# arkCyber/whisper-rust

Hardware: AMD Instinct MI355X
Metric: real-time factor (audio-sec/wall-sec), greedy, 30 s synthetic chunks (higher is better)
Workload: dtype f16 operands / f32 accumulate; 1 GPU; ggml-small-shaped synthetic F16 model, greedy best_of=1 temperature_inc=0, 1 x 30 s 16 kHz f32 chunk per GPU, PCM resident in HBM; flash_attn=False, parallelism=chunk-dp1

## Files before the change

### whisper-rust_amd/csrc/wa_mega.hip

```cpp
#include "wa_device.h"
#include "wa_mega.h"

typedef unsigned long long u64;
#define GAS __attribute__((address_space(1)))
typedef GAS u64 gu64;
typedef GAS unsigned gu32;
typedef const GAS wa_f16 * gch;
typedef const GAS float * gcf;
typedef _Float16 half4v __attribute__((ext_vector_type(4)));
typedef unsigned u32x2 __attribute__((ext_vector_type(2)));
typedef unsigned u32x4 __attribute__((ext_vector_type(4)));

typedef const __attribute__((address_space(4))) wa_mega_args * mg_kargs;
__device__ __forceinline__ mg_kargs mg_uniform(mg_kargs p) {
    const unsigned long long v = (unsigned long long) p;
    const unsigned lo = __builtin_amdgcn_readfirstlane((unsigned) v), hi = __builtin_amdgcn_readfirstlane((unsigned) (v >> 32));
    return (mg_kargs) (((unsigned long long) hi << 32) | lo);
}

#define MG_THREADS 512
#define MG_NW (MG_THREADS / 64)
#define MG_NP3 4
#define MG_SPIN_LIMIT 20000u
#ifndef MG_DEFER
// ... 776 lines not shown
            }
            mg_trace(A, wg == 0 && own && lane == 0, (l * 8 + 1) * 8 + 3, mg_now());
            if (A->dbg && l == MG_WGTRACE_LAYER) mg_trace(A, own && lane == 0, 1024 + wg * 8 + 3, mg_now());
            if (own && !MG_DEFER) t = mg_mk8<Q, NS>(pf, Y.co_w, Y.co_d, Y.co_b, nullptr, d, d, row_d, r_d, 0, lane);
            else if (assisted) t = mg_mk16<Q, 4 * NS>(pf, Y.fc2_w, Y.fc2_d, Y.fc2_b, d, d4, row_d, r_d, 0, lane);
        }
        MG_FRESH();
        if constexpr (CQ) {
            const int qs = mg_slot(wave, MG_EX_X1), sg = mg_seg(d), i0 = qs * sg, i1 = min(d, i0 + sg);
            if (qs >= 0) mg_gather_f32<NP3>(c, mg_edge(A, l, E_X1), i0, i1, lane, xf, 300u + l, A,
                                            wave == 0 ? (wg == 0 ? (l * 8 + 2) * 8 : (A->dbg && l == MG_WGTRACE_LAYER ? 1024 + wg * 8 : -1)) : -1);
            mg_barrier();
            MG_FRESH();
            if (wave == 4) t = mg_mk8<Q, NS>(pf, Y.co_w, Y.co_d, Y.co_b, nullptr, d, d, row_d, r_d, 0, lane);
            else if (wave == 3 || wave >= 6) {
                if (l + 1 >= L) mg_prefetch_logits<NS, Q>(A, pf, have_pf, lane, wave);
                else if (wave == 3) t = mg_mk8<Q, NS>(pf, Ly[l + 1].out_w, Ly[l + 1].out_d, Ly[l + 1].out_b, nullptr, d, d, row_d, r_d, 0, lane);
                else t = mg_mk8<Q, NS>(pf, Ly[l + 1].qkv_w, Ly[l + 1].qkv_d, Ly[l + 1].qkv_b, Ly[l + 1].qkv_s, 3 * d, d, row_qkv, r_qkv, wave - 6, lane);
            }
        } else
        mg_ln3<NP3, Q>(A, c, mg_edge(A, l, E_X1), gw, gb, mg_slot(wave, MG_EX_P4), lane, xf, xinB, lnred, 300u + l,
                       wave == 0 ? (wg == 0 ? (l * 8 + 2) * 8 : (A->dbg && l == MG_WGTRACE_LAYER ? 1024 + wg * 8 : -1)) : -1);
        MG_FRESH();
        if (MG_DEFER && !CQ && wave == 3) t = mg_mk8<Q, NS>(pf, Y.co_w, Y.co_d, Y.co_b, nullptr, d, d, row_d, r_d, 0, lane);
        if (BIGP && wave >= 6 && wave - 2 < g_ff) t = mg_mk8<Q, NS>(pf, Y.fc1_w, Y.fc1_d, Y.fc1_b, nullptr, d4, d, row_ff, r_ff, wave - 2, lane);
        mg_ln_params<NP3>(gw, gb, Y.ln3_w, Y.ln3_b, d, mg_slot(wave, MG_EX_P7), lane);
        if (!CQ && (wave == 4 || (BIG && wave == 3))) {
            const bool own = !BIG || wave == 4;
            bool assisted = false;
            gu64 * eq = mg_edge(A, l, E_QC);
            for (int grp = own ? 0 : 1; grp < g_d8; grp += BIG ? 2 : 1) {
                if (grp >= 1) { t = mg_mk8<Q, NS>(pf, Y.cq_w, Y.cq_d, Y.cq_b, nullptr, d, d, row_d, r_d, grp, lane); assisted = true; }
                MG_CHAOS_AT(3u);
                float v = mg_do8<Q, NS>(pf, t, d >> 5, xinB, lane);
                v = v + t.bias;
                mg_pub_h2(eq, seq, t.valid, t.row, (unsigned) f2h(v), lane);
            }
            mg_trace(A, wg == 0 && own && lane == 0, (l * 8 + 2) * 8 + 3, mg_now());
            if (A->dbg && l == MG_WGTRACE_LAYER) mg_trace(A, own && lane == 0, 1024 + wg * 8 + 6, mg_now());
            if (QB) t = mg_mk8<Q, NS>(pf, Y.fc1_w, Y.fc1_d, Y.fc1_b, nullptr, d4, d, 32 * wg, 32, 3, lane);
            else if (own && !MG_DEFER) {
                if (l + 1 < L) t = mg_mk8<Q, NS>(pf, Ly[l + 1].cq_w, Ly[l + 1].cq_d, Ly[l + 1].cq_b, nullptr, d, d, row_d, r_d, 0, lane);
                else mg_prefetch_logits<NS, Q>(A, pf, have_pf, lane, wave);
            } else if (assisted) t = mg_mk8<Q, NS>(pf, Y.co_w, Y.co_d, Y.co_b, nullptr, d, d, row_d, r_d, 0, lane);
        }
        MG_FRESH();
        {
            const int qs = mg_slot(wave, MG_EX_AO2), sg = mg_seg(Q ? 9 * (d >> 5) : d >> 1), j0 = qs * sg, j1 = min(Q ? 9 * (d >> 5) : d >> 1, j0 + sg);
            if constexpr (Q) { if (qs >= 0) mg_gather_qb<1>(c, mg_edge(A, l, E_AO2), j0, j1, lane, xin, d >> 5, 400u + l, A, wg == 0 && wave == 0 ? (l * 8 + 3) * 8 : -1); }
            else if (qs >= 0) mg_gather_h2<2>(c, mg_edge(A, l, E_AO2), j0, j1, lane, (unsigned *) xin, 400u + l, A, wg == 0 && wave == 0 ? (l * 8 + 3) * 8 : -1);
        }
        mg_barrier();
        MG_FRESH();
        if (MG_DEFER && !QB && !BIGP && !CQ && wave == 4) {
            if (l + 1 < L) t = mg_mk8<Q, NS>(pf, Ly[l + 1].cq_w, Ly[l + 1].cq_d, Ly[l + 1].cq_b, nullptr, d, d, row_d, r_d, 0, lane);
            else mg_prefetch_logits<NS, Q>(A, pf, have_pf, lane, wave);
        }
        if (wave == (CQ ? 4 : 3) || (BIG && wave == 4)) {
            const bool own = !BIG || wave == 3;
            bool assisted = false;
            gu64 * ex = mg_edge(A, l, E_X2);
            for (int grp = own ? 0 : 1; grp < g_d8; grp += BIG ? 2 : 1) {
                if (grp >= 1) { t = mg_mk8<Q, NS>(pf, Y.co_w, Y.co_d, Y.co_b, nullptr, d, d, row_d, r_d, grp, lane); assisted = true; }
                MG_CHAOS_AT(4u);
                float v = mg_do8<Q, NS>(pf, t, d >> 5, xin, lane);
                v = v + t.bias;
                if (t.valid && (lane & 7) == 0) gr_store(ex + t.row, seq, __float_as_uint(v + xf[t.row]));
            }
            mg_trace(A, wg == 0 && own && lane == 0, (l * 8 + 3) * 8 + 3, mg_now());
            if (A->dbg && l == MG_WGTRACE_LAYER) mg_trace(A, own && lane == 0, 4096 + wg * 8 + 3, mg_now());
            if (QB) t = mg_mk8<Q, NS>(pf, Y.fc1_w, Y.fc1_d, Y.fc1_b, nullptr, d4, d, 32 * wg, 32, 2, lane);
            else if (CQ) { if (l + 1 >= L) mg_prefetch_logits<NS, Q>(A, pf, have_pf, lane, wave); }
            else if (BIGP) {
                if (wave - 1 < g_ff) t = mg_mk8<Q, NS>(pf, Y.fc1_w, Y.fc1_d, Y.fc1_b, nullptr, d4, d, row_ff, r_ff, wave - 1, lane);
                else big_next(wave);
            } else if (own && !MG_DEFER) {
                if (l + 1 < L) t = mg_mk8<Q, NS>(pf, Ly[l + 1].out_w, Ly[l + 1].out_d, Ly[l + 1].out_b, nullptr, d, d, row_d, r_d, 0, lane);
                else mg_prefetch_logits<NS, Q>(A, pf, have_pf, lane, wave);
            } else if (assisted) {
                if (l + 1 < L) t = mg_mk8<Q, NS>(pf, Ly[l + 1].cq_w, Ly[l + 1].cq_d, Ly[l + 1].cq_b, nullptr, d, d, row_d, r_d, 0, lane);
                else mg_prefetch_logits<NS, Q>(A, pf, have_pf, lane, wave);
            }
        }
        MG_FRESH();
        if (l == 0 && wave >= 3 && wave <= 5) asm volatile("s_waitcnt vmcnt(0)" ::: "memory");
        mg_ln3<NP3, Q>(A, c, mg_edge(A, l, E_X2), gw, gb, mg_slot(wave, MG_EX_P7), lane, xf, xinB, lnred, 500u + l,
                       wave == 0 ? (wg == 0 ? (l * 8 + 4) * 8 : (A->dbg && l == MG_WGTRACE_LAYER ? 4096 + wg * 8 : -1)) : -1);
        MG_FRESH();
        if (MG_DEFER && !QB && !BIGP && !CQ && wave == 3) {
            if (l + 1 < L) t = mg_mk8<Q, NS>(pf, Ly[l + 1].out_w, Ly[l + 1].out_d, Ly[l + 1].out_b, nullptr, d, d, row_d, r_d, 0, lane);
            else mg_prefetch_logits<NS, Q>(A, pf, have_pf, lane, wave);
        }
        if (l + 1 < L) mg_ln_params<NP3>(gw, gb, Ly[l + 1].ln1_w, Ly[l + 1].ln1_b, d, mg_slot(wave, MG_EX_P1), lane);
        else           mg_ln_params<NP3>(gw, gb, A->lnf_w, A->lnf_b, d, mg_slot(wave, MG_EX_FINAL), lane);
        if (QB) {
            if (wave >= 1 && wave <= 4) {
                MG_CHAOS_AT(5u);
                float v = mg_do8<Q, NS>(pf, t, d >> 5, xinB, lane);
                v = v + t.bias;
                float gl = v;
                if (v <= -10.0f) gl = 0.0f; else if (v < 10.0f) gl = h2f(gelu_l[t.valid ? f2h(v) : 0]);
                if ((lane & 7) == 0) fc1x[8 * (wave - 1) + (lane >> 3)] = gl;
                MG_CHAOS_AT(51u);
                unsigned arrived = 0;
                asm volatile("s_waitcnt lgkmcnt(0)" ::: "memory");
                if (lane == 0) arrived = __hip_atomic_fetch_add(fc1cnt, 1u, __ATOMIC_RELAXED, __HIP_MEMORY_SCOPE_WORKGROUP);
                arrived = (unsigned) __builtin_amdgcn_readfirstlane((int) arrived);
                asm volatile("" ::: "memory");
                if ((arrived & 3u) == 3u && 32 * wg < d4) {
                    MG_CHAOS_AT(52u);
                    const float y = fc1x[lane & 31];
                    float a = fabsf(y);
                    a = fmaxf(a, dpp_f32<0x128>(a)); a = fmaxf(a, dpp_f32<0x124>(a)); a = fmaxf(a, dpp_f32<0x122>(a)); a = fmaxf(a, dpp_f32<0x121>(a));
                    a = fmaxf(a, __shfl_xor(a, 16, 32));
                    const float dq = a / 127.f, id = a != 0.0f ? 127.f / a : 0.0f;
                    const unsigned q = (unsigned) (int) rintf(y * id) & 0xffu;
                    const unsigned w = q | (dpp_u32<0x101>(q) << 8) | (dpp_u32<0x102>(q) << 16) | (dpp_u32<0x103>(q) << 24);
                    gu64 * eb = mg_edge(A, l, E_HF) + (size_t) wg * 9;
                    if (lane < 32 && (lane & 3) == 0) gr_store(eb + (lane >> 2), seq, w);
                    if (lane == 0) gr_store(eb + 8, seq, __float_as_uint(h2f(f2h(dq))));
                    mg_trace(A, wg == 0 && lane == 0, (l * 8 + 4) * 8 + 3, mg_now());
                }
                if (wave == 3) {
                    if (l + 1 < L) t = mg_mk8<Q, NS>(pf, Ly[l + 1].out_w, Ly[l + 1].out_d, Ly[l + 1].out_b, nullptr, d, d, row_d, r_d, 0, lane);
                    else mg_prefetch_logits<NS, Q>(A, pf, have_pf, lane, wave);
                } else if (wave == 4) {
                    if (l + 1 < L) t = mg_mk8<Q, NS>(pf, Ly[l + 1].cq_w, Ly[l + 1].cq_d, Ly[l + 1].cq_b, nullptr, d, d, row_d, r_d, 0, lane);
                    else mg_prefetch_logits<NS, Q>(A, pf, have_pf, lane, wave);
                }
            }
        } else if (BIGP) {
            if ((wave >= 1 && wave <= 4) || wave >= 6) {
                gu64 * eh = mg_edge(A, l, E_HF);
                for (int grp = wave <= 4 ? wave - 1 : wave - 2; grp < g_ff; grp += 6) {
                    if (grp >= 6) t = mg_mk8<Q, NS>(pf, Y.fc1_w, Y.fc1_d, Y.fc1_b, nullptr, d4, d, row_ff, r_ff, grp, lane);
                    MG_CHAOS_AT(6u);
                    float v = mg_do8<Q, NS>(pf, t, d >> 5, xinB, lane);
                    v = v + t.bias;
                    float gl = v;
                    if (v <= -10.0f) gl = 0.0f; else if (v < 10.0f) gl = h2f(gelu_l[t.valid ? f2h(v) : 0]);
                    if constexpr (Q) { if (t.valid && (lane & 7) == 0) gr_store(eh + t.row, seq, __float_as_uint(gl)); }
                    else mg_pub_h2(eh, seq, t.valid, t.row, (unsigned) f2h(gl), lane);
                }
                mg_trace(A, wg == 0 && wave == 1 && lane == 0, (l * 8 + 4) * 8 + 3, mg_now());
                if ((wave == 3 || wave == 4) && wave - 1 < g_ff) big_next(wave);
                else if (wave >= 6 && l + 1 >= L) mg_prefetch_logits<NS, Q>(A, pf, have_pf, lane, wave);
            }
        } else
        if (wave == 1 || wave == 2 || (BIG && (wave == 3 || wave == 4))) {
            const bool own = !BIG || wave <= 2;
            bool assisted = false;
            gu64 * eh = mg_edge(A, l, E_HF);
            for (int grp = wave - 1; grp < g_ff; grp += BIG ? 4 : 2) {
                if (grp >= 2) { t = mg_mk8<Q, NS>(pf, Y.fc1_w, Y.fc1_d, Y.fc1_b, nullptr, d4, d, row_ff, r_ff, grp, lane); assisted = true; }
                MG_CHAOS_AT(7u);
                float v = mg_do8<Q, NS>(pf, t, d >> 5, xinB, lane);
                v = v + t.bias;
                float gl = v;
                if (v <= -10.0f) gl = 0.0f; else if (v < 10.0f) gl = h2f(gelu_l[t.valid ? f2h(v) : 0]);
                if constexpr (Q) { if (t.valid && (lane & 7) == 0) gr_store(eh + t.row, seq, __float_as_uint(gl)); }
                else mg_pub_h2(eh, seq, t.valid, t.row, (unsigned) f2h(gl), lane);
            }
            mg_trace(A, wg == 0 && wave == 1 && lane == 0, (l * 8 + 4) * 8 + 3, mg_now());
            if (A->dbg && l == MG_WGTRACE_LAYER) mg_trace(A, wave == 1 && lane == 0, 4096 + wg * 8 + 6, mg_now());
            if (own && !MG_DEFER) {
                if (l + 1 < L) t = mg_mk8<Q, NS>(pf, Ly[l + 1].qkv_w, Ly[l + 1].qkv_d, Ly[l + 1].qkv_b, Ly[l + 1].qkv_s, 3 * d, d, row_qkv, r_qkv, wave - 1, lane);
                else mg_prefetch_logits<NS, Q>(A, pf, have_pf, lane, wave);
            } else if (CQ) {
                if (l + 1 >= L) mg_prefetch_logits<NS, Q>(A, pf, have_pf, lane, wave);
            } else if (assisted) {
                if (l + 1 >= L) mg_prefetch_logits<NS, Q>(A, pf, have_pf, lane, wave);
                else t = wave == 3 ? mg_mk8<Q, NS>(pf, Ly[l + 1].out_w, Ly[l + 1].out_d, Ly[l + 1].out_b, nullptr, d, d, row_d, r_d, 0, lane)
                                   : mg_mk8<Q, NS>(pf, Ly[l + 1].cq_w, Ly[l + 1].cq_d, Ly[l + 1].cq_b, nullptr, d, d, row_d, r_d, 0, lane);
            }
        }
        MG_FRESH();
        {
            const int ng = QB ? 9 * (d4 >> 5) : Q ? d4 : 2 * d;
            const int qs = mg_slot(wave, QB || BIGP ? MG_EX_HFQ : MG_EX_HF), sg = mg_seg(ng), i0 = qs * sg, i1 = min(ng, i0 + sg);
            if constexpr (QB) { if (qs >= 0) mg_gather_qb<3>(c, mg_edge(A, l, E_HF), i0, i1, lane, xin, d4 >> 5, 600u + l, A, wg == 0 && wave == 0 ? (l * 8 + 5) * 8 : -1); }
            else if constexpr (Q) { if (qs >= 0) mg_gather_q8<(NP3 == MG_NP3 ? 14 : 8)>(c, mg_edge(A, l, E_HF), i0, i1, lane, xin, d4 >> 5, 600u + l, A, wg == 0 && wave == 0 ? (l * 8 + 5) * 8 : -1); }
            else if (qs >= 0) mg_gather_h2<7>(c, mg_edge(A, l, E_HF), i0, i1, lane, (unsigned *) xin, 600u + l, A, wg == 0 && wave == 0 ? (l * 8 + 5) * 8 : -1);
        }
        mg_barrier();
        MG_FRESH();
        mg_trace(A, wg == 0 && wave == 5 && lane == 0, (l * 8 + 5) * 8 + 4, mg_now());
        if (MG_DEFER && !CQ && (wave == 1 || wave == 2)) {
            if (l + 1 < L) t = mg_mk8<Q, NS>(pf, Ly[l + 1].qkv_w, Ly[l + 1].qkv_d, Ly[l + 1].qkv_b, Ly[l + 1].qkv_s, 3 * d, d, row_qkv, r_qkv, wave - 1, lane);
            else mg_prefetch_logits<NS, Q>(A, pf, have_pf, lane, wave);
        }
        if (wave == 5 || (BIG && (wave == 3 || wave == 4))) {
            const bool own = !BIG || wave == 5;
            bool assisted = false;
            gu64 * ex = mg_edge(A, l, E_X3);
            for (int grp = own ? 0 : wave - 2; grp < g_d16; grp += BIG ? 3 : 1) {
                if (grp >= (BIGP ? 3 : 1)) t = mg_mk16<Q, 4 * NS>(pf, Y.fc2_w, Y.fc2_d, Y.fc2_b, d, d4, row_d, r_d, grp, lane);
                if (grp >= 1) assisted = true;
                MG_CHAOS_AT(8u);
                float v = mg_do16<Q, 4 * NS>(pf, t, d4 >> 5, xin, lane);
                v = v + t.bias;
                if (t.valid && (lane & 15) == MG_RES16(Q)) gr_store(ex + t.row, seq, __float_as_uint(v + xf[t.row]));
            }
            mg_trace(A, wg == 0 && own && lane == 0, (l * 8 + 5) * 8 + 3, mg_now());
            if (own && (!MG_DEFER || l + 1 >= L)) {
                if (l + 1 < L) t = mg_mk16<Q, 4 * NS>(pf, Ly[l + 1].fc2_w, Ly[l + 1].fc2_d, Ly[l + 1].fc2_b, d, d4, row_d, r_d, 0, lane);
                else mg_prefetch_logits<NS, Q>(A, pf, have_pf, lane, wave);
            } else if (assisted) {
                if (l + 1 >= L) mg_prefetch_logits<NS, Q>(A, pf, have_pf, lane, wave);
                else t = wave == 3 ? mg_mk8<Q, NS>(pf, Ly[l + 1].out_w, Ly[l + 1].out_d, Ly[l + 1].out_b, nullptr, d, d, row_d, r_d, 0, lane)
                                   : mg_mk8<Q, NS>(pf, Ly[l + 1].cq_w, Ly[l + 1].cq_d, Ly[l + 1].cq_b, nullptr, d, d, row_d, r_d, 0, lane);
            }
        }
    }
    if (L == 0 && wave >= 1 && wave <= 5) mg_prefetch_logits<NS, Q>(A, pf, have_pf, lane, wave);
    MG_FRESH();
    mg_final<NP3, NS, Q>(A, c, smem, pf, have_pf, gw, gb, lane, wave);
#undef MG_FRESH
}

struct mg_att_smem { float * sc; wa_f16 * p16; float * gs; float * red; double * redd; float * s_inv; wa_f16 * qs; float * part; };
__device__ __forceinline__ mg_att_smem mg_att_carve(unsigned char * base, int maxkv) {
    mg_att_smem m;
    m.redd = (double *) base;                       base += 8 * sizeof(double);
    m.sc   = (float *) base;                        base += (size_t) maxkv * 4;
    m.gs   = (float *) base;                        base += (size_t) (maxkv / 8) * 4;
    m.part = (float *) base;                        base += 32 * 64 * 4;
    m.red  = (float *) base;                        base += 8 * 4;
    m.s_inv = (float *) base;                       base += 4 * 4;
    m.p16  = (wa_f16 *) base;                       base += (size_t) maxkv * 2;
    m.qs   = (wa_f16 *) base;
    return m;
}


__device__ __forceinline__ float mg_score(const u32x4 & ka, const u32x4 & kb, const float (&qa)[8], const float (&qb)[8], float scale) {
    const wa_f16 * k8a = (const wa_f16 *) &ka, * k8b = (const wa_f16 *) &kb;
    float v[8];
#pragma unroll
    for (int l = 0; l < 8; ++l) {
        float t = fmaf(h2f(k8a[l]), qa[l], 0.0f);
        t = fmaf(h2f(k8b[l]), qb[l], t);
        t = t + dpp_f32<0x4e>(t);
        v[l] = t + dpp_f32<0xb1>(t);
    }
    const float t0 = v[0] + v[4], t1 = v[1] + v[5], t2 = v[2] + v[6], t3 = v[3] + v[7];
    return ((t0 + t1) + (t2 + t3)) * scale;
}

template <bool Q = false>
__device__ __forceinline__ void mg_attn_finish(const float * part, const wa_f16 * vleft , const wa_f16 * p16, int np, int nl,
                                               gu64 * edge, int h, unsigned seq, int tid, double * dbl0, double * dbl1 ,
                                               mg_kargs A = nullptr, int tslot = -1) {
    asm volatile("" : "+s"(nl));
    if (tid >= 64) {
        const int wv = tid >> 6, o = tid & 63;
        float nzero = -0.0f;
        asm volatile("" : "+v"(nzero));
#pragma unroll
        for (int i = 0; i < 5; ++i) {
            const int cc = 5 * (wv - 1) + i;
            if (cc < 32) {
                const float pr = fmaf(h2f(vleft[cc * 64 + o]), h2f((p16 + np)[cc]), nzero);
                (cc < 16 ? dbl0 : dbl1)[(cc & 15) * 64 + o] = (double) (cc < nl ? pr : -0.0f);
            }
        }
    }
    double sumf = 0.0;
    if (tid < 64) {
        if (tslot >= 0) mg_trace(A, tid == 0, tslot, mg_now());
        float s32[32];
#pragma unroll
        for (int r = 0; r < 32; ++r) s32[r] = part[r * 64 + tid];
        sumf = (double) wa_tree32(s32);
        if (tslot >= 0) mg_trace(A, tid == 0, tslot + 1, mg_now() + (sumf == 1e300 ? 1u : 0u));
    }
    mg_barrier();
    if (tid < 64) {
        double dv[32];
#pragma unroll
        for (int cc = 0; cc < 32; ++cc) dv[cc] = (cc < 16 ? dbl0 : dbl1)[(cc & 15) * 64 + tid];
        __builtin_amdgcn_sched_barrier(0);
#pragma unroll
        for (int cc = 0; cc < 32; ++cc) sumf += dv[cc];
        if (tslot >= 0) mg_trace(A, tid == 0, tslot + 2, mg_now() + (sumf == 1e300 ? 1u : 0u));
        if constexpr (Q) {
            const float y = (float) sumf;
            float a = fabsf(y);
            a = fmaxf(a, dpp_f32<0x128>(a)); a = fmaxf(a, dpp_f32<0x124>(a)); a = fmaxf(a, dpp_f32<0x122>(a)); a = fmaxf(a, dpp_f32<0x121>(a));
            a = fmaxf(a, __shfl_xor(a, 16, 32));
            const float dsc = a / 127.f, id = a != 0.0f ? 127.f / a : 0.0f;
            const unsigned q = (unsigned) (int) rintf(y * id) & 0xffu;
            const unsigned w = q | (dpp_u32<0x101>(q) << 8) | (dpp_u32<0x102>(q) << 16) | (dpp_u32<0x103>(q) << 24);
            gu64 * eb = edge + (size_t) (2 * h + (tid >> 5)) * 9;
            if ((tid & 3) == 0) gr_store(eb + ((tid & 31) >> 2), seq, w);
            if ((tid & 31) == 0) gr_store(eb + 8, seq, __float_as_uint(h2f(f2h(dsc))));
        } else {
        const unsigned hv = (unsigned) f2h((float) sumf);
        const unsigned hi = dpp_u32<0x101>(hv);
        if ((tid & 1) == 0) gr_store(edge + ((h * 64 + tid) >> 1), seq, (hv & 0xffffu) | (hi << 16));
        }
    }
}

template <bool Q = false>
__device__ __forceinline__ void mg_role_self(mg_kargs A_, int idx_) {
    extern __shared__ __attribute__((aligned(16))) unsigned char smem[];
    const mg_kargs A = mg_uniform(A_);
    const int tid = threadIdx.x, lane = tid & 63;
    const int wave = __builtin_amdgcn_readfirstlane(tid >> 6);
    const int h = __builtin_amdgcn_readfirstlane(idx_);
    mg_ctl c; c.status = (gu32 *) A->status; c.seq = A->seq; c.dead = false;
    mg_chaos_start(c.seq);

    wa_f16 * Ks = (wa_f16 *) smem;
    wa_f16 * Vs = Ks + WA_MEGA_MAX_KV * 64;
    const mg_att_smem M = mg_att_carve(smem + (size_t) WA_MEGA_MAX_KV * 64 * 2 * 2, WA_MEGA_MAX_KV);
    const int d = A->d, n_kv = A->n_kv, kv_head = A->kv_head, L = A->n_layer;
    const int a = tid & 3, kslot = tid >> 2;
    if (wave == 0) mg_pick(A, lane, (int *) (smem + MG_PICK_OFF));
    for (int l = 0; l < L; ++l) {
        {
            const gch kc = (gch) A->kv_k + (size_t) l * A->kv_layer_stride + h * 64;
            const gch vc = (gch) A->kv_v + (size_t) l * A->kv_layer_stride + h * 64;
            const int n16 = n_kv * 8;
            u32x4 tk[8], tv[8];
#pragma unroll
            for (int j = 0; j < 8; ++j) {
                const int idx = tid + MG_THREADS * j;
                if (idx < n16) {
                    tk[j] = *(const GAS u32x4 *) (kc + (size_t) (idx >> 3) * d + (idx & 7) * 8);
                    tv[j] = *(const GAS u32x4 *) (vc + (size_t) (idx >> 3) * d + (idx & 7) * 8);
                }
            }
#pragma unroll
            for (int j = 0; j < 8; ++j) {
                const int idx = tid + MG_THREADS * j;
                if (idx < n16) { *(u32x4 *) (Ks + (size_t) idx * 8) = tk[j]; *(u32x4 *) (Vs + (size_t) idx * 8) = tv[j]; }
            }
        }
        mg_barrier();
        if (wave == 0) {
            unsigned v[2];
            const unsigned sp = mg_sweep<2>(mg_edge(A, l, E_QKV), [&](int k) {
                if (k == 0) return (lane < 32 ? 0 : (d >> 1)) + h * 32 + (lane & 31);
                return lane < 32 ? d + h * 32 + lane : -1; }, c, lane, v, 1000u + l);
            mg_trace(A, h == 0 && lane == 0, (l * 8 + 6) * 8 + 0, mg_now()); mg_trace(A, h == 0 && lane == 0, (l * 8 + 6) * 8 + 1, sp);
            if (lane < 32) { ((unsigned *) M.qs)[lane] = v[0]; ((unsigned *) (Vs + (size_t) kv_head * 64))[lane] = v[1]; }
            else ((unsigned *) (Ks + (size_t) kv_head * 64))[lane - 32] = v[0];
        }
        mg_barrier();
        float lmax = -INFINITY;
        {
            float qa[8], qb[8];
#pragma unroll
            for (int i = 0; i < 8; ++i) { qa[i] = h2f(M.qs[8 * a + i]); qb[i] = h2f(M.qs[32 + 8 * a + i]); }
            for (int c0 = 0; c0 < n_kv; c0 += MG_THREADS / 4) {
                const int cc = c0 + kslot, cl = cc < n_kv ? cc : n_kv - 1;
                const u32x4 ka = *(const u32x4 *) (Ks + (size_t) cl * 64 + 8 * a), kb = *(const u32x4 *) (Ks + (size_t) cl * 64 + 32 + 8 * a);
                const float r = mg_score(ka, kb, qa, qb, 1.0f);
                if (cc < n_kv) { if (a == 0) M.sc[cc] = r; lmax = fmaxf(lmax, r); }
            }
        }
        mg_trace(A, h == 0 && tid == 0, (l * 8 + 6) * 8 + 4, mg_now());
        {
            lmax = wave_max(lmax);
            if (lane == 0) M.red[wave] = lmax;
            mg_barrier();
            float mx = M.red[0];
#pragma unroll
            for (int k = 1; k < MG_NW; ++k) mx = fmaxf(mx, M.red[k]);
            const int n8 = n_kv & ~7, ng = n8 >> 3;
            float e = 0.0f;
            double ps = 0.0;
            if (tid < n_kv) e = tid < n8 ? wa_expf(M.sc[tid] - mx) : wa_expf_libm(M.sc[tid] - mx);
            {
                float t = e + dpp_f32<0x104>(e);
                t = t + dpp_f32<0x102>(t);
                t = t + dpp_f32<0x101>(t);
                if (tid < n8) ps = (tid & 7) == 0 ? (double) t : 0.0;
                else if (tid < n_kv) ps = (double) e;
            }
            ps = wave_sum_d(ps);
            if (lane == 0) M.redd[wave] = ps;
            mg_barrier();
            const double tot = ((M.redd[0] + M.redd[1]) + (M.redd[2] + M.redd[3])) + ((M.redd[4] + M.redd[5]) + (M.redd[6] + M.redd[7]));
            const double delta = (double) (ng + 8 + 16) * 0x1p-53 * tot * 1.000001;
            const float ilo = (float) (1.0 / (tot + delta)), ihi = (float) (1.0 / (tot - delta));
            if (ilo != ihi && tid == 0 && !c.dead) __hip_atomic_store(c.status, (unsigned) WA_MEGA_REDO, __ATOMIC_RELAXED, __HIP_MEMORY_SCOPE_AGENT);
            if (tid < n_kv) M.p16[tid] = f2h(e * ilo);
            mg_barrier();
        }
        mg_trace(A, h == 0 && tid == 0, (l * 8 + 6) * 8 + 5, mg_now());
        MG_CHAOS_ID(1000 + h, 21u, c.seq);
        const int np = n_kv & ~31, nsteps = np >> 5;
        {
            float acc[4] = { 0.0f, 0.0f, 0.0f, 0.0f };
            const int r0 = wave * 4;
            for (int s = 0; s < nsteps; ++s) {
#pragma unroll
                for (int i = 0; i < 4; ++i)
                    acc[i] = fmaf(h2f(Vs[(size_t) (s * 32 + r0 + i) * 64 + lane]), h2f(M.p16[s * 32 + r0 + i]), acc[i]);
            }
#pragma unroll
            for (int i = 0; i < 4; ++i) M.part[(r0 + i) * 64 + lane] = acc[i];
        }
        mg_barrier();
        mg_attn_finish<Q>(M.part, Vs + (size_t) np * 64, M.p16, np, n_kv - np, mg_edge(A, l, E_AO), h, c.seq, tid, (double *) (Ks + WA_MEGA_KV_ROOM * 64),
                          (double *) (Vs + WA_MEGA_KV_ROOM * 64), A, A->dbg && h == 0 && l == MG_WGTRACE_LAYER ? 3004 : -1);
        mg_trace(A, h == 0 && tid == 0, (l * 8 + 6) * 8 + 3, mg_now());
        mg_barrier();
    }
    unsigned pf[96];
    bool have_pf = false;
    float gw[MG_NP3], gb[MG_NP3];
    if (wave >= 1) mg_prefetch_logits<0, Q>(A, pf, have_pf, lane, wave);
    mg_ln_params<MG_NP3>(gw, gb, A->lnf_w, A->lnf_b, A->d, mg_slot(wave, MG_EX_FINAL), lane);
    mg_final<MG_NP3, 0, Q>(A, c, smem, pf, have_pf, gw, gb, lane, wave);
}

#define MG_CSTEPS 48
#define MG_CGR 2048
#define MG_CGR_MAX 0
#define MG_CGR_SUM 8
#define MG_CGR_XCC 16
#define MG_CGR_PART 64
#define MG_CX_XF 32768
#define MG_CX_XIN (MG_CX_XF + WA_MEGA_MAX_D * 4)
#define MG_CX_LNRED (MG_CX_XIN + WA_MEGA_MAX_D * 2)
#define MG_CX_END (MG_CX_LNRED + 256)
#define MG_CX_TRACE 6144

template <bool Q = false, int CQ = -1>
__device__ __forceinline__ void mg_role_cross(mg_kargs A_, int idx_) {
    extern __shared__ __attribute__((aligned(16))) unsigned char smem[];
    const mg_kargs A = mg_uniform(A_);
    int tid = threadIdx.x, lane = tid & 63;
    const int wave = __builtin_amdgcn_readfirstlane(tid >> 6);
    const int H = A->n_head;
    const int ci = __builtin_amdgcn_readfirstlane(idx_);
    const int h = ci >> 2, w = ci & 3;
    mg_ctl c; c.status = (gu32 *) A->status; c.seq = A->seq; c.dead = false;
    mg_chaos_start(c.seq);
    const unsigned seq = c.seq;

    float  * part  = (float *) smem;
    wa_f16 * vleft = (wa_f16 *) (smem + 8192);
    float  * sc    = (float *) (smem + 8192 + 4096);
    wa_f16 * p16   = (wa_f16 *) (smem + 8192 + 4096 + 1536);
    wa_f16 * pleft = (wa_f16 *) (smem + 8192 + 4096 + 1536 + 768);
    wa_f16 * qs    = (wa_f16 *) (smem + 8192 + 4096 + 1536 + 768 + 64);
    double * redd  = (double *) (smem + 8192 + 4096 + 1536 + 768 + 64 + 128);
    float  * red   = (float *) (smem + 8192 + 4096 + 1536 + 768 + 64 + 128 + 64);
    float  * bc    = red + 8;

    const int T = A->T, tpad = A->cross_tpad, L = A->n_layer;
    const float kq_scale = A->kq_scale;
    int a = tid & 3, ks = tid >> 2;
    const int np = T & ~31, nsteps = np >> 5, nl = T - np, n8 = T & ~7, ng = n8 >> 3;
    if (wave == 0) mg_pick(A, lane, (int *) (smem + MG_PICK_OFF));
    if (wave == 0) {
        const unsigned xcc = (unsigned) __builtin_amdgcn_s_getreg(20 | (3 << 11)) & 0xfu;
        gu64 * X0 = (gu64 *) A->cross_gr + (size_t) h * MG_CGR + MG_CGR_XCC;
        if (lane == 0) gr_store(X0 + w, seq, xcc);
        unsigned v[1];
        mg_sweep<1>(X0, [&](int) { return lane < 4 ? lane : -1; }, c, lane, v, 2900u);
        const bool same = lane >= 4 || v[0] == xcc;
        if (lane == 0) bc[2] = __builtin_amdgcn_ballot_w64(same) == ~0ull && !c.dead ? 1.0f : 0.0f;
    }
    mg_barrier();
    const bool local = bc[2] != 0.0f;
    const __attribute__((address_space(4))) wa_mega_layer * Ly = (const __attribute__((address_space(4))) wa_mega_layer *) A->layers;
    float  * xf    = (float *) (smem + MG_CX_XF);
    wa_f16 * xin   = (wa_f16 *) (smem + MG_CX_XIN);
    double * lnred = (double *) (smem + MG_CX_LNRED);
    const int d = A->d;
    for (int l = 0; l < L; ++l) {
        if constexpr (CQ >= 0) {
            unsigned z = threadIdx.x; asm volatile("" : "+v"(z));
            tid = (int) z; lane = tid & 63; a = tid & 3; ks = tid >> 2;
        }
        gu64 * X = (gu64 *) A->cross_gr + ((size_t) l * H + h) * MG_CGR;
        const gch kp = (gch) A->cross_k + (size_t) l * A->cross_layer_stride + (size_t) h * tpad * 64;
        const gch vp = (gch) A->cross_v + (size_t) l * A->cross_layer_stride + (size_t) h * tpad * 64;
        u32x4 ka[3], kb[3];
        unsigned short vv[MG_CSTEPS];
#pragma unroll
        for (int p = 0; p < 3; ++p) {
            const int o = p * 128 + ks, cc = 32 * (o >> 3) + 8 * w + (o & 7);
            if (cc < T) { ka[p] = *(const GAS u32x4 *) (kp + (size_t) cc * 64 + 8 * a); kb[p] = *(const GAS u32x4 *) (kp + (size_t) cc * 64 + 32 + 8 * a); }
        }
#pragma unroll
        for (int s = 0; s < MG_CSTEPS; ++s) if (s < nsteps) vv[s] = *(const GAS unsigned short *) (vp + (size_t) (32 * s + 8 * w + wave) * 64 + lane);
        if (w == 0 && tid < 256) {
            const int row = tid >> 3;
            if (row < nl) *(u32x4 *) (vleft + (size_t) tid * 8) = *(const GAS u32x4 *) (vp + (size_t) (np + row) * 64 + (tid & 7) * 8);
        }
        if constexpr (CQ >= 0) {
            unsigned pf[96];
            float gw[2], gb[2];
            const int row = 64 * h + 8 * wave + (lane >> 3);
            const gch wrow = (gch) Ly[l].cq_w + (size_t) row * d + 4 * (lane & 7);
            mg_pf8<CQ>(pf, wrow, true, d >> 5, 0);
            const float bias = ((gcf) Ly[l].cq_b)[row];
            mg_ln_params<2>(gw, gb, Ly[l].ln2_w, Ly[l].ln2_b, d, mg_slot(wave, 0u), lane);
            mg_trace(A, ci == 0 && lane == 0 && wave == 0, (l * 8 + 7) * 8 + 2, mg_now());
            mg_ln3<2>(A, c, mg_edge(A, l, E_X1), gw, gb, mg_slot(wave, 0u), lane, xf, xin, lnred, 2000u + l,
                      ci == 0 && wave == 0 ? MG_CX_TRACE + l * 8 : -1);
            MG_CHAOS_ID(2000 + ci, 30u, seq);
            float v = mg_dot8<CQ>(pf, wrow, true, d >> 5, xin, lane & 7, true);
            v = v + bias;
            const unsigned hq = (unsigned) f2h(v);
            if ((lane & 7) == 0) qs[8 * wave + (lane >> 3)] = (wa_f16) hq;
            if (A->dbg && w == 0) mg_pub_h2(mg_edge(A, l, E_QC), seq, true, row, hq, lane);
            mg_trace(A, ci == 0 && lane == 0 && wave == 0, (l * 8 + 7) * 8 + 0, mg_now());
            if (A->dbg && l == MG_WGTRACE_LAYER && w == 0) mg_trace(A, tid == 0, 3200 + h, mg_now());
        } else if (wave == 0) {
            unsigned v[1];
            mg_trace(A, ci == 0 && lane == 0, (l * 8 + 7) * 8 + 2, mg_now());
            const unsigned sp = mg_sweep<1>(mg_edge(A, l, E_QC), [&](int) { return lane < 32 ? h * 32 + lane : -1; }, c, lane, v, 2000u + l);
            mg_trace(A, ci == 0 && lane == 0, (l * 8 + 7) * 8 + 0, mg_now()); mg_trace(A, ci == 0 && lane == 0, (l * 8 + 7) * 8 + 1, sp);
            if (A->dbg && l == MG_WGTRACE_LAYER && w == 0) mg_trace(A, lane == 0, 3200 + h, mg_now());
            if (lane < 32) ((unsigned *) qs)[lane] = v[0];
        }
        mg_barrier();
#define MG_CX(k) do { if (A->dbg && l == MG_WGTRACE_LAYER) mg_trace(A, ci == 0 && tid == 0, 3010 + (k), mg_now()); } while (0)
        MG_CX(0);
        MG_CHAOS_ID(2000 + ci, 31u, seq);
        float lmax = -INFINITY;
        {
            float qa[8], qb[8];
#pragma unroll
            for (int i = 0; i < 8; ++i) { qa[i] = h2f(qs[8 * a + i]); qb[i] = h2f(qs[32 + 8 * a + i]); }
#pragma unroll
            for (int p = 0; p < 3; ++p) {
                const int o = p * 128 + ks, cc = 32 * (o >> 3) + 8 * w + (o & 7);
                const float r = mg_score(ka[p], kb[p], qa, qb, kq_scale);
                if (cc < T) { if (a == 0) sc[o] = r; lmax = fmaxf(lmax, r); }
            }
        }
        lmax = wave_max(lmax);
        if (lane == 0) red[wave] = lmax;
        MG_CX(1);
        mg_barrier();
        MG_CX(2);
        if (wave == 0) {
            float m = red[0];
#pragma unroll
            for (int k = 1; k < MG_NW; ++k) m = fmaxf(m, red[k]);
            if (lane == 0) gr_store_l(X + MG_CGR_MAX + w, seq, __float_as_uint(m), local);
            unsigned v[1];
            mg_sweep<1>(X + MG_CGR_MAX, [&](int) { return lane < 4 ? lane : -1; }, c, lane, v, 2100u + l);
            float g = lane < 4 ? __uint_as_float(v[0]) : -INFINITY;
            g = fmaxf(g, dpp_f32<0x4e>(g)); g = fmaxf(g, dpp_f32<0xb1>(g));
            if (lane == 0) bc[0] = g;
            MG_CX(3);
        }
        mg_barrier();
        mg_trace(A, ci == 0 && tid == 0, (l * 8 + 7) * 8 + 4, mg_now());
        const float mx = bc[0];
        {
            double ps = 0.0;
            if (tid < 8 * MG_CSTEPS) {
                const int g = 4 * (tid >> 3) + w, cc = 8 * g + (tid & 7);
                const float e = cc < n8 ? wa_expf(sc[tid] - mx) : (cc < T ? wa_expf_libm(sc[tid] - mx) : 0.0f);
                sc[tid] = e;
                float t = e + dpp_f32<0x104>(e);
                t = t + dpp_f32<0x102>(t);
                t = t + dpp_f32<0x101>(t);
                if (g < ng) ps = (tid & 7) == 0 ? (double) t : 0.0;
                else ps = (double) e;
            }
            ps = wave_sum_d(ps);
            if (lane == 0) redd[wave] = ps;
        }
        MG_CX(4);
        mg_barrier();
        if (wave == 0) {
            const double ps = ((redd[0] + redd[1]) + (redd[2] + redd[3])) + ((redd[4] + redd[5]) + (redd[6] + redd[7]));
            const u64 pb = (u64) __double_as_longlong(ps);
            if (lane == 0) { gr_store_l(X + MG_CGR_SUM + 2 * w, seq, (unsigned) pb, local); gr_store_l(X + MG_CGR_SUM + 2 * w + 1, seq, (unsigned) (pb >> 32), local); }
            unsigned v[1];
            mg_sweep<1>(X + MG_CGR_SUM, [&](int) { return lane < 8 ? lane : -1; }, c, lane, v, 2200u + l);
            double tot = 0.0;
#pragma unroll
            for (int k = 0; k < 4; ++k) {
                const unsigned lo = __builtin_amdgcn_readlane(v[0], 2 * k), hi = __builtin_amdgcn_readlane(v[0], 2 * k + 1);
                tot += __longlong_as_double((long long) (((u64) hi << 32) | lo));
            }
            const double delta = (double) (ng + 8 + 16) * 0x1p-53 * tot * 1.000001;
            const float ilo = (float) (1.0 / (tot + delta)), ihi = (float) (1.0 / (tot - delta));
            if (ilo != ihi && lane == 0 && !c.dead) __hip_atomic_store(c.status, (unsigned) WA_MEGA_REDO, __ATOMIC_RELAXED, __HIP_MEMORY_SCOPE_AGENT);
            if (lane == 0) bc[1] = ilo;
            MG_CX(5);
        }
        mg_barrier();
        mg_trace(A, ci == 0 && tid == 0, (l * 8 + 7) * 8 + 5, mg_now());
        const float inv = bc[1];
        if (tid < 8 * MG_CSTEPS) {
            const int cc = 32 * (tid >> 3) + 8 * w + (tid & 7);
            if (cc < T) {
                const wa_f16 ph = f2h(sc[tid] * inv);
                p16[(tid & 7) * MG_CSTEPS + (tid >> 3)] = ph;
                if (cc >= np) { if (w == 0) pleft[cc - np] = ph; else gr_store_l(X + MG_CGR_PART + (w - 1) * 576 + 512 + (tid & 7), seq, (unsigned) ph, local); }
            }
        }
        mg_barrier();
        MG_CX(6);
        MG_CHAOS_ID(2000 + ci, 32u, seq);
        {
            float acc = 0.0f;
            half8 pw[MG_CSTEPS / 8];
#pragma unroll
            for (int k = 0; k < MG_CSTEPS / 8; ++k) pw[k] = *(const half8 *) (p16 + wave * MG_CSTEPS + 8 * k);
#pragma unroll
            for (int s = 0; s < MG_CSTEPS; ++s) if (s < nsteps) acc = fmaf(h2f(vv[s]), (float) pw[s >> 3][s & 7], acc);
            if (w == 0) part[wave * 64 + lane] = acc;
            else gr_store_l(X + MG_CGR_PART + (w - 1) * 576 + wave * 64 + lane, seq, __float_as_uint(acc), local);
        }
        mg_trace(A, ci == 0 && tid == 0, (l * 8 + 7) * 8 + 6, mg_now());
        if (w == 0) {
            if (wave >= 1 && wave <= 6) {
                const int ww = (wave - 1) >> 1, half = (wave - 1) & 1;
                gu64 * src = X + MG_CGR_PART + ww * 576;
                unsigned v[5];
                mg_sweep<5>(src, [&](int k) { return k < 4 ? half * 256 + 64 * k + lane : (half == 0 && lane < 8 && 8 * (ww + 1) + lane < nl ? 512 + lane : -1); }, c, lane, v, 2300u + l);
#pragma unroll
                for (int k = 0; k < 4; ++k) part[(8 * (ww + 1) + 4 * half + k) * 64 + lane] = __uint_as_float(v[k]);
                if (half == 0 && lane < 8) { const int cc = 8 * (ww + 1) + lane; if (cc < nl) pleft[cc] = (wa_f16) v[4]; }
            }
            mg_barrier();
            mg_trace(A, ci == 0 && tid == 0, (l * 8 + 7) * 8 + 7, mg_now());
            mg_attn_finish<Q>(part, vleft, pleft - np, np, nl, mg_edge(A, l, E_AO2), h, seq, tid, (double *) (smem + 16384), (double *) (smem + 24576), A,
                              A->dbg && ci == 0 && l == MG_WGTRACE_LAYER ? 3000 : -1);
            mg_trace(A, ci == 0 && tid == 0, (l * 8 + 7) * 8 + 3, mg_now());
            if (A->dbg && l == MG_WGTRACE_LAYER) mg_trace(A, tid == 0, 3100 + h, mg_now());
        }
        mg_barrier();
    }
    unsigned pf[96];
    bool have_pf = false;
    float gw[MG_NP3], gb[MG_NP3];
    if (wave >= 1) mg_prefetch_logits<0, Q>(A, pf, have_pf, lane, wave);
    mg_ln_params<MG_NP3>(gw, gb, A->lnf_w, A->lnf_b, A->d, mg_slot(wave, MG_EX_FINAL), lane);
    mg_final<MG_NP3, 0, Q>(A, c, smem, pf, have_pf, gw, gb, lane, wave);
}

#ifndef MG_CQ_TU
__global__ __launch_bounds__(MG_THREADS) void k_decode_mega(const wa_mega_args A) {
    int role, idx;
    mg_role_of((int) gridDim.x, A.n_head, (int) blockIdx.x, role, idx);
    const mg_kargs Ap = (mg_kargs) __builtin_amdgcn_kernarg_segment_ptr();
    if (role == 0) {
        if (A.d == 768) mg_role_gemv<2, 24>(Ap, idx); else if (A.d < 768) mg_role_gemv<2, 0>(Ap, idx);
        else mg_role_gemv<MG_NP3, 0>(Ap, idx);
    }
    else if (role == 1) mg_role_self(Ap, idx);
    else                mg_role_cross(Ap, idx);
}


__global__ __launch_bounds__(MG_THREADS) void k_decode_mega_q(const wa_mega_args A) {
    int role, idx;
    mg_role_of((int) gridDim.x, A.n_head, (int) blockIdx.x, role, idx);
    const mg_kargs Ap = (mg_kargs) __builtin_amdgcn_kernarg_segment_ptr();
    if (role == 0) {
        if (A.d == 768) mg_role_gemv<2, 24, true>(Ap, idx); else if (A.d < 768) mg_role_gemv<2, 0, true>(Ap, idx);
        else if (A.d == 1280) mg_role_gemv<MG_NP3, 40, true>(Ap, idx); else mg_role_gemv<MG_NP3, 0, true>(Ap, idx);
    }
    else if (role == 1) mg_role_self<true>(Ap, idx);
    else                mg_role_cross<true>(Ap, idx);
}

size_t wa_mega_lds_bytes() {
    const size_t s_self  = (size_t) WA_MEGA_MAX_KV * 64 * 2 * 2 + MG_ATT_SMEM(WA_MEGA_MAX_KV);
    const size_t s_cross = MG_CX_END;
    const size_t s_gemv  = MG_PICK_OFF;
    size_t m = s_self > s_cross ? s_self : s_cross;
    m = m > s_gemv ? m : s_gemv;
    if (m > MG_PICK_OFF || (MG_PICK_OFF & 255) != 0) abort();
    return MG_PICK_OFF + MG_PICK_BYTES;
}

bool wa_launch_decode_mega(hipStream_t s, const wa_mega_args & a, int n_wg) {
    static bool attr_set[64] = {};
    const size_t lds = wa_mega_lds_bytes();
    int dev = 0;
    (void) hipGetDevice(&dev);
    if (!attr_set[dev & 63]) {
        if (hipFuncSetAttribute((const void *) k_decode_mega, hipFuncAttributeMaxDynamicSharedMemorySize, (int) lds) != hipSuccess ||
            hipFuncSetAttribute((const void *) k_decode_mega_q, hipFuncAttributeMaxDynamicSharedMemorySize, (int) lds) != hipSuccess) return false;
        attr_set[dev & 63] = true;
    }
    if (MG_DEFER && !a.quant && a.d == 768) return wa_launch_decode_mega_cq(s, a, n_wg, lds);
    if (a.quant) hipLaunchKernelGGL(k_decode_mega_q, dim3(n_wg), dim3(MG_THREADS), lds, s, a);
    else         hipLaunchKernelGGL(k_decode_mega, dim3(n_wg), dim3(MG_THREADS), lds, s, a);
    return hipGetLastError() == hipSuccess;
}
#else
__global__ __launch_bounds__(MG_THREADS) void k_decode_mega_cq(const wa_mega_args A) {
    int role, idx;
    mg_role_of((int) gridDim.x, A.n_head, (int) blockIdx.x, role, idx);
    const mg_kargs Ap = (mg_kargs) __builtin_amdgcn_kernarg_segment_ptr();
    if (role == 0)      mg_role_gemv<2, 24, false, true>(Ap, idx);
    else if (role == 1) mg_role_self(Ap, idx);
    else                mg_role_cross<false, 24>(Ap, idx);
}

bool wa_launch_decode_mega_cq(hipStream_t s, const wa_mega_args & a, int n_wg, size_t lds) {
    static bool attr_set[64] = {};
    int dev = 0;
    (void) hipGetDevice(&dev);
    if (!attr_set[dev & 63]) {
        if (hipFuncSetAttribute((const void *) k_decode_mega_cq, hipFuncAttributeMaxDynamicSharedMemorySize, (int) lds) != hipSuccess) return false;
        attr_set[dev & 63] = true;
    }
    hipLaunchKernelGGL(k_decode_mega_cq, dim3(n_wg), dim3(MG_THREADS), lds, s, a);
    return hipGetLastError() == hipSuccess;
}
#endif
```

Baseline: 350.5 x real-time.

## Split cross-attention V columns across the four workgroups to need one exchange

```diff
diff --git a/whisper-rust_amd/csrc/wa_mega.hip b/whisper-rust_amd/csrc/wa_mega.hip
--- a/whisper-rust_amd/csrc/wa_mega.hip
+++ b/whisper-rust_amd/csrc/wa_mega.hip
@@ -1102,6 +1102,28 @@
     }
 }
 
+__device__ __forceinline__ void mg_attn_finish16(const float * part, const double * dbl, gu64 * edge, int o0, unsigned seq, int tid,
+                                                 mg_kargs A = nullptr, int tslot = -1) {
+    if (tid < 16) {
+        if (tslot >= 0) mg_trace(A, tid == 0, tslot, mg_now());
+        float s32[32];
+        double dv[32];
+#pragma unroll
+        for (int r = 0; r < 32; ++r) s32[r] = part[r * 16 + tid];
+#pragma unroll
+        for (int cc = 0; cc < 32; ++cc) dv[cc] = dbl[cc * 16 + tid];
+        __builtin_amdgcn_sched_barrier(0);
+        double sumf = (double) wa_tree32(s32);
+        if (tslot >= 0) mg_trace(A, tid == 0, tslot + 1, mg_now() + (sumf == 1e300 ? 1u : 0u));
+#pragma unroll
+        for (int cc = 0; cc < 32; ++cc) sumf += dv[cc];
+        if (tslot >= 0) mg_trace(A, tid == 0, tslot + 2, mg_now() + (sumf == 1e300 ? 1u : 0u));
+        const unsigned hv = (unsigned) f2h((float) sumf);
+        const unsigned hi = dpp_u32<0x101>(hv);
+        if ((tid & 1) == 0) gr_store(edge + ((o0 + tid) >> 1), seq, (hv & 0xffffu) | (hi << 16));
+    }
+}
+
 template <bool Q = false>
 __device__ __forceinline__ void mg_role_self(mg_kargs A_, int idx_) {
     extern __shared__ __attribute__((aligned(16))) unsigned char smem[];
@@ -1224,14 +1246,17 @@
 #define MG_CGR_SUM 8
 #define MG_CGR_XCC 16
 #define MG_CGR_PART 64
+#define MG_CGR_XCC1 WA_MEGA_MAX_T
+#define MG_CP_LD 56
 #define MG_CX_XF 32768
 #define MG_CX_XIN (MG_CX_XF + WA_MEGA_MAX_D * 4)
 #define MG_CX_LNRED (MG_CX_XIN + WA_MEGA_MAX_D * 2)
 #define MG_CX_END (MG_CX_LNRED + 256)
 #define MG_CX_TRACE 6144
 
-template <bool Q = false, int CQ = -1>
+template <bool Q = false, int CQ = -1, bool X1 = false>
 __device__ __forceinline__ void mg_role_cross(mg_kargs A_, int idx_) {
+    static_assert(!X1 || (CQ >= 0 && !Q), "the one-exchange form is the F16 d = 768 kernel's");
     extern __shared__ __attribute__((aligned(16))) unsigned char smem[];
     const mg_kargs A = mg_uniform(A_);
     int tid = threadIdx.x, lane = tid & 63;
@@ -1252,6 +1277,23 @@
     double * redd  = (double *) (smem + 8192 + 4096 + 1536 + 768 + 64 + 128);
     float  * red   = (float *) (smem + 8192 + 4096 + 1536 + 768 + 64 + 128 + 64);
     float  * bc    = red + 8;
+    double * dbl   = nullptr;
+    if constexpr (X1) {
+        constexpr int o_sc = 0, o_p16 = o_sc + WA_MEGA_MAX_T * 4, o_part = o_p16 + 32 * MG_CP_LD * 2, o_dbl = o_part + 32 * 16 * 4, o_vleft = o_dbl + 32 * 16 * 8,
+                      o_pleft = o_vleft + 32 * 16 * 2, o_qs = o_pleft + 32 * 2, o_redd = o_qs + 64 * 2, o_red = o_redd + 8 * 8, o_bc = o_red + 8 * 4, o_end = o_bc + 4 * 4;
+        static_assert(o_end <= MG_CX_XF && o_p16 % 16 == 0 && o_dbl % 8 == 0 && o_vleft % 16 == 0 && o_redd % 8 == 0 && MG_CP_LD % 8 == 0 && MG_CP_LD >= MG_CSTEPS,
+                      "LDS of the one-exchange form: below the role's LayerNorm area, 16-byte rows where 16 bytes are read");
+        sc    = (float *) (smem + o_sc);
+        p16   = (wa_f16 *) (smem + o_p16);
+        part  = (float *) (smem + o_part);
+        dbl   = (double *) (smem + o_dbl);
+        vleft = (wa_f16 *) (smem + o_vleft);
+        pleft = (wa_f16 *) (smem + o_pleft);
+        qs    = (wa_f16 *) (smem + o_qs);
+        redd  = (double *) (smem + o_redd);
+        red   = (float *) (smem + o_red);
+        bc    = (float *) (smem + o_bc);
+    }
 
     const int T = A->T, tpad = A->cross_tpad, L = A->n_layer;
     const float kq_scale = A->kq_scale;
@@ -1260,7 +1302,7 @@
     if (wave == 0) mg_pick(A, lane, (int *) (smem + MG_PICK_OFF));
     if (wave == 0) {
         const unsigned xcc = (unsigned) __builtin_amdgcn_s_getreg(20 | (3 << 11)) & 0xfu;
-        gu64 * X0 = (gu64 *) A->cross_gr + (size_t) h * MG_CGR + MG_CGR_XCC;
+        gu64 * X0 = (gu64 *) A->cross_gr + (size_t) h * MG_CGR + (X1 ? MG_CGR_XCC1 : MG_CGR_XCC);
         if (lane == 0) gr_store(X0 + w, seq, xcc);
         unsigned v[1];
         mg_sweep<1>(X0, [&](int) { return lane < 4 ? lane : -1; }, c, lane, v, 2900u);
@@ -1289,11 +1331,20 @@
             const int o = p * 128 + ks, cc = 32 * (o >> 3) + 8 * w + (o & 7);
             if (cc < T) { ka[p] = *(const GAS u32x4 *) (kp + (size_t) cc * 64 + 8 * a); kb[p] = *(const GAS u32x4 *) (kp + (size_t) cc * 64 + 32 + 8 * a); }
         }
+        if constexpr (X1) {
+#pragma unroll
+            for (int s = 0; s < MG_CSTEPS; ++s) if (s < nsteps) vv[s] = *(const GAS unsigned short *) (vp + (size_t) (32 * s + (tid >> 4)) * 64 + 16 * w + (tid & 15));
+            if (wave == 0) {
+                const int row = tid >> 1;
+                if (row < nl) *(u32x4 *) (vleft + (size_t) tid * 8) = *(const GAS u32x4 *) (vp + (size_t) (np + row) * 64 + 16 * w + (tid & 1) * 8);
+            }
+        } else {
 #pragma unroll
         for (int s = 0; s < MG_CSTEPS; ++s) if (s < nsteps) vv[s] = *(const GAS unsigned short *) (vp + (size_t) (32 * s + 8 * w + wave) * 64 + lane);
         if (w == 0 && tid < 256) {
             const int row = tid >> 3;
             if (row < nl) *(u32x4 *) (vleft + (size_t) tid * 8) = *(const GAS u32x4 *) (vp + (size_t) (np + row) * 64 + (tid & 7) * 8);
+        }
         }
         if constexpr (CQ >= 0) {
             unsigned pf[96];
@@ -1324,6 +1375,107 @@
         }
         mg_barrier();
 #define MG_CX(k) do { if (A->dbg && l == MG_WGTRACE_LAYER) mg_trace(A, ci == 0 && tid == 0, 3010 + (k), mg_now()); } while (0)
+        if constexpr (X1) {
+        MG_CX(0);
+        MG_CHAOS_ID(2000 + ci, 31u, seq);
+        float lmax = -INFINITY;
+        {
+            float qa[8], qb[8];
+#pragma unroll
+            for (int i = 0; i < 8; ++i) { qa[i] = h2f(qs[8 * a + i]); qb[i] = h2f(qs[32 + 8 * a + i]); }
+#pragma unroll
+            for (int p = 0; p < 3; ++p) {
+                const int o = p * 128 + ks, cc = 32 * (o >> 3) + 8 * w + (o & 7);
+                const float r = mg_score(ka[p], kb[p], qa, qb, kq_scale);
+                if (cc < T) {
+                    if (a == 0) { gr_store_l(X + cc, seq, __float_as_uint(r), local); sc[cc] = r; }
+                    lmax = fmaxf(lmax, r);
+                }
+            }
+        }
+        MG_CX(1);
+        MG_CHAOS_ID(2000 + ci, 33u, seq);
+        {
+            unsigned v[3];
+            const auto other = [&](int k) { const int cg = tid + 512 * k; return cg < T && ((cg >> 3) & 3) != w ? cg : -1; };
+            mg_sweep<3>(X, other, c, lane, v, 2400u + l);
+#pragma unroll
+            for (int k = 0; k < 3; ++k) {
+                const int cg = other(k);
+                if (cg >= 0) { const float r = __uint_as_float(v[k]); sc[cg] = r; lmax = fmaxf(lmax, r); }
+            }
+        }
+        lmax = wave_max(lmax);
+        if (lane == 0) red[wave] = lmax;
+        MG_CX(2);
+        mg_barrier();
+        MG_CX(3);
+        mg_trace(A, ci == 0 && tid == 0, (l * 8 + 7) * 8 + 4, mg_now());
+        MG_CHAOS_ID(2000 + ci, 34u, seq);
+        float mx = red[0];
+#pragma unroll
+        for (int k = 1; k < MG_NW; ++k) mx = fmaxf(mx, red[k]);
+        float e[3];
+        {
+            double ps = 0.0;
+#pragma unroll
+            for (int k = 0; k < 3; ++k) {
+                const int cg = tid + 512 * k, g = cg >> 3;
+                const float sv = sc[cg];
+                e[k] = cg < n8 ? wa_expf(sv - mx) : (cg < T ? wa_expf_libm(sv - mx) : 0.0f);
+                float t = e[k] + dpp_f32<0x104>(e[k]);
+                t = t + dpp_f32<0x102>(t);
+                t = t + dpp_f32<0x101>(t);
+                ps += g < ng ? ((tid & 7) == 0 ? (double) t : 0.0) : (double) e[k];
+            }
+            ps = wave_sum_d(ps);
+            if (lane == 0) redd[wave] = ps;
+        }
+        MG_CX(4);
+        mg_barrier();
+        mg_trace(A, ci == 0 && tid == 0, (l * 8 + 7) * 8 + 5, mg_now());
+        {
+            const double tot = ((redd[0] + redd[1]) + (redd[2] + redd[3])) + ((redd[4] + redd[5]) + (redd[6] + redd[7]));
+            const double delta = (double) (ng + 8 + 16) * 0x1p-53 * tot * 1.000001;
+            const float ilo = (float) (1.0 / (tot + delta)), ihi = (float) (1.0 / (tot - delta));
+            if (ilo != ihi && tid == 0 && !c.dead) __hip_atomic_store(c.status, (unsigned) WA_MEGA_REDO, __ATOMIC_RELAXED, __HIP_MEMORY_SCOPE_AGENT);
+#pragma unroll
+            for (int k = 0; k < 3; ++k) {
+                const int cg = tid + 512 * k;
+                if (cg < T) {
+                    const wa_f16 ph = f2h(e[k] * ilo);
+                    if (cg < np) p16[(cg & 31) * MG_CP_LD + (cg >> 5)] = ph;
+                    else pleft[cg - np] = ph;
+                }
+            }
+        }
+        MG_CX(5);
+        mg_barrier();
+        MG_CX(6);
+        MG_CHAOS_ID(2000 + ci, 32u, seq);
+        {
+            const int r = tid >> 4;
+            float acc = 0.0f;
+            half8 pw[MG_CSTEPS / 8];
+#pragma unroll
+            for (int k = 0; k < MG_CSTEPS / 8; ++k) pw[k] = *(const half8 *) (p16 + r * MG_CP_LD + 8 * k);
+#pragma unroll
+            for (int s = 0; s < MG_CSTEPS; ++s) if (s < nsteps) acc = fmaf(h2f(vv[s]), (float) pw[s >> 3][s & 7], acc);
+            part[tid] = acc;
+            float nzero = -0.0f;
+            asm volatile("" : "+v"(nzero));
+            int nlo = nl;
+            asm volatile("" : "+s"(nlo));
+            const float pr = fmaf(h2f(vleft[tid]), h2f(pleft[r]), nzero);
+            dbl[tid] = (double) (r < nlo ? pr : -0.0f);
+        }
+        mg_trace(A, ci == 0 && tid == 0, (l * 8 + 7) * 8 + 6, mg_now());
+        mg_barrier();
+        mg_trace(A, ci == 0 && tid == 0, (l * 8 + 7) * 8 + 7, mg_now());
+        mg_attn_finish16(part, dbl, mg_edge(A, l, E_AO2), 64 * h + 16 * w, seq, tid, A, A->dbg && ci == 0 && l == MG_WGTRACE_LAYER ? 3000 : -1);
+        mg_trace(A, ci == 0 && tid == 0, (l * 8 + 7) * 8 + 3, mg_now());
+        if (A->dbg && l == MG_WGTRACE_LAYER && w == 0) mg_trace(A, tid == 0, 3100 + h, mg_now());
+        } else {
         MG_CX(0);
         MG_CHAOS_ID(2000 + ci, 31u, seq);
         float lmax = -INFINITY;
@@ -1435,6 +1587,7 @@
             mg_trace(A, ci == 0 && tid == 0, (l * 8 + 7) * 8 + 3, mg_now());
             if (A->dbg && l == MG_WGTRACE_LAYER) mg_trace(A, tid == 0, 3100 + h, mg_now());
         }
+        }
         mg_barrier();
     }
     unsigned pf[96];
@@ -1503,7 +1656,7 @@
     const mg_kargs Ap = (mg_kargs) __builtin_amdgcn_kernarg_segment_ptr();
     if (role == 0)      mg_role_gemv<2, 24, false, true>(Ap, idx);
     else if (role == 1) mg_role_self(Ap, idx);
-    else                mg_role_cross<false, 24>(Ap, idx);
+    else                mg_role_cross<false, 24, true>(Ap, idx);
 }
 
 bool wa_launch_decode_mega_cq(hipStream_t s, const wa_mega_args & a, int n_wg, size_t lds) {
```

Result: faster. 359.9 x real-time (median of 6 runs) (+2.7%).
